# nitishthatte/QuadrotorILQR

Hardware: AMD Instinct MI355X
Metric: iLQR solves/sec (batch, 100-knot SE(3) quadrotor) (higher is better)
Workload: dtype f64

## Files before the change

### profiles/microbench/round_stamps.py

```python
#!/usr/bin/env python3
import ctypes as C, os, sys
import numpy as np
ROOT = os.path.dirname(os.path.dirname(os.path.dirname(os.path.abspath(__file__))))
sys.path.insert(0, ROOT)
from quadrotorilqr_amd import capi, problems as pb
capi.LIB_PATH = os.path.join(ROOT, "quadrotorilqr_amd", "lib", "libquadrotor_ilqr_roundstamps.so")
B = int(sys.argv[1]) if len(sys.argv) > 1 else 1024
cfg = pb.config2(B=B, N=100, seed=2)
s = capi.from_config(cfg)
s.solve_batch(cfg["init"])
lib = capi.load()
zero = np.zeros((max(B, 8) * 8,), dtype=np.uint64)
lib.qilqr_debug_stamps(s._h, zero.ctypes.data_as(C.c_void_p), C.c_int32(B))
out0 = zero.copy()
res = s.solve_batch(cfg["init"])
lib.qilqr_debug_stamps(s._h, zero.ctypes.data_as(C.c_void_p), C.c_int32(B))
d = (zero - out0).reshape(-1, 32)[: (B + 3) // 4, :4].astype(np.float64)
rounds = d[:, 3]
ok = rounds > 0
live_rounds = np.add.reduceat(np.asarray(res["n_fwd"], dtype=np.float64), np.arange(0, B, 4))
print(f"B = {B}: blocks {ok.sum()}, rounds per block (median) {np.median(rounds[ok]):.0f}, in ticks of s_memtime / 100")
for name, k in (("backward pass", 0), ("rollout (until X_0 is through)", 1), ("behind the rollout", 2)):
    per = d[ok, k] / rounds[ok]
    print(f"  {name:32s} median {np.median(per) / 100:7.2f} us per round   (p10 {np.percentile(per, 10) / 100:.2f}, p90 {np.percentile(per, 90) / 100:.2f})")
dense = live_rounds[ok] / rounds[ok]
for lo, hi in ((0.9, 1.5), (1.5, 2.5), (2.5, 4.1)):
    m = (dense >= lo) & (dense < hi)
    if m.sum():
        tot = d[ok][m, :3].sum(axis=1) / rounds[ok][m]
        print(f"  blocks with {lo:.1f}-{hi:.1f} running trajectories per round on average: {m.sum():4d} blocks, {np.median(tot) / 100:7.2f} us per round "
              f"(backward {np.median(d[ok][m, 0] / rounds[ok][m]) / 100:.2f}, rollout {np.median(d[ok][m, 1] / rounds[ok][m]) / 100:.2f}, behind {np.median(d[ok][m, 2] / rounds[ok][m]) / 100:.2f})")
```

### quadrotorilqr_amd/csrc/backward4_body.inc

```
  const int lane = threadIdx.x & 63;
  const int w = __builtin_amdgcn_readfirstlane((int)(threadIdx.x >> 6));
  const int b0 = xcd_local_block(blockIdx.x, gridDim.x) * 4;
#ifndef BW4_LDS_DECLARED
  BW4_DECLARE_LDS
#endif
  if (FREE && threadIdx.x < 24) prog[threadIdx.x] = (threadIdx.x >= 8) ? -1 : 0;
  const RecLayout L = st.layout;

  double mu = 0.0;
  if (w < 4) {
    const int b = b0 + w;
    bool run = false;
    int cur = 0, iters_now = 0, act = 0;
    double cost_now = 0.0;
    if (b < B) {
      int fl = st.flags[b];
      cur = st.cur[b];
      const int it0 = st.iters[b];
      const int trial0 = st.trial[b];
      const double prev_cost0 = st.prev_cost[b], alpha0 = st.alpha[b];
      const double term0 = st.terms[2 * b], term1 = st.terms[2 * b + 1];
      cost_now = st.cost[b];
      const int n_fwd0 = st.n_fwd[b];
      mu = (p.mu_init > 0.0) ? st.mu[b] : 0.0;
      double kc_early[2][2];
#pragma unroll
      for (int h = 0; h < 2; ++h)
#pragma unroll
        for (int k = 0; k < 2; ++k) {
          const int i = 64 * h + lane;
          kc_early[k][h] = (i < n) ? st.knot_cost[k][cost_index(b, i, n)] : 0.0;
        }
      bool restart = false;
      bool settle = false, accept = false, count_active = false, known = true;
      int status = -1;
      double new_cost = 0.0;
      if (!force) {
        if (fl & F_SEARCH) {
          settle = true;
          const double *kc = st.knot_cost[cur ^ 1];
          double *scr = &ring[w][0][0];
          auto add_chunk = [&](double v, int cnt) {
            scr[lane] = v;
            int t = 0;
            for (; t + 8 <= cnt; t += 8) {
              double x[8];
#pragma unroll
              for (int e = 0; e < 8; ++e) x[e] = scr[t + e];
#pragma unroll
              for (int e = 0; e < 8; ++e) new_cost += x[e];
            }
            for (; t < cnt; ++t) new_cost += scr[t];
          };
          add_chunk((cur ^ 1) ? kc_early[1][0] : kc_early[0][0], n < 64 ? n : 64);
          if (n > 64) add_chunk((cur ^ 1) ? kc_early[1][1] : kc_early[0][1], n < 128 ? n - 64 : 64);
          for (int base = 128; base < n; base += 64) {
            const int i = base + lane;
            add_chunk((i < n) ? kc[cost_index(b, i, n)] : 0.0, (n - base < 64) ? n - base : 64);
          }
          if (it0 == 0) {
            accept = true;
          } else {
            const double desired = p.reduction_frac * cost_reduction(term0, term1, alpha0);
            accept = (new_cost - prev_cost0 < desired);
          }
          if (accept) {
            cur ^= 1;
            fl = F_ACTIVE;
            cost_now = new_cost;
            mu = lm_relax(p, mu);
            if (it0 > 0 && is_converged(p, prev_cost0, new_cost)) {
              status = 1;
              fl = 0;
            } else if (!((double)(it0 + 1) < p.max_iters)) {
              status = 2;
              fl = 0;
            }
          } else if (trial0 + 1 >= p.ls_max_iters) {
            if (lm_restart(p, mu)) {
              restart = true;
              fl = F_ACTIVE;
            } else {
              status = 3;
              fl = 0;
            }
          }
          count_active = (fl & F_ACTIVE) != 0;
        } else if (fl == F_ACTIVE) {
          count_active = true;
        } else {
          known = false;
        }
      }
      run = known && (force || !settle || ((accept || restart) && fl != 0));
      iters_now = (settle && accept) ? it0 + 1 : it0;
      if (lane == 0 && known) {
        if (settle) {
          if (p.mu_init > 0.0) st.mu[b] = mu;
          st.n_fwd[b] = n_fwd0 + 1;
          store_settled(st, b, accept, cur, new_cost, it0, trial0, alpha0, p.step_update, status, fl);
        }
        act = count_active ? 1 : 0;
      }
    }
    if (lane == 0) {
      s_act[w] = act;
      s_run[w] = run ? 1 : 0;
      s_cur[w] = cur;
      s_iters[w] = iters_now;
      s_cost[w] = cost_now;
      s_mu[w] = mu;
    }
  }
  __syncthreads();
  const int block_act = s_act[0] + s_act[1] + s_act[2] + s_act[3];
  if ((s_run[0] | s_run[1] | s_run[2] | s_run[3]) == 0) {
    if (threadIdx.x == 0 && block_act) atomicAdd(active_counter(st), block_act);
    BW4_RETURN;
  }

#ifndef BW4_CTAB_FILLED
  bw4_fill_ctab<S>(ring, st.ctab, FUSED ? 320 : 384);
#endif
  if (!FUSED && w == 4) {
    const int g = lane >> 4, j = lane & 15;
    const int bg = (b0 + g < B) ? b0 + g : B - 1;
    const bool grun = s_run[g] != 0;
    double QuTk;
    if constexpr (GFAC) {
      const double cuu_ab = 2.0 * c.R[(j >> 2) * 4 + (j & 3)] + (((j >> 2) == (j & 3)) ? s_mu[g] : 0.0);
      QuTk = bw4f_gradient_wave<S>(ring, kf, kw, L, (S *)st.gains + knot_base<true>(bg, n, 52), (S *)st.dump + 4 * (long)bg, grun, cuu_ab, n, lane);
    } else {
      QuTk = bw4_gradient_wave<S>(ring, kf, L, (S *)st.gains + knot_base<true>(bg, n, 52), (S *)st.dump + 4 * (long)bg, grun, n, lane);
    }
    if (j == 0 && grun) {
      const int b = b0 + g;
      st.terms[2 * b] = QuTk;
      st.terms[2 * b + 1] = -QuTk;
      st.n_bwd[b] += 1;
      if (!force) arm_line_search(p, st, b, s_iters[g], s_cost[g], QuTk, -QuTk);
    }
    if (lane == 0 && block_act) atomicAdd(active_counter(st), block_act);
    BW4_RETURN;
  }

  if (w == (FUSED ? 4 : 5)) {
    const int first = s_run[0] ? 0 : (s_run[1] ? 1 : (s_run[2] ? 2 : 3));
    const S *rec[4];
#pragma unroll
    for (int g = 0; g < 4; ++g) {
      const int gs = s_run[g] ? g : first;
      rec[g] = (const S *)st.lin[s_cur[gs]] + rec_base(L, b0 + gs, n);
    }
    bw4_loader_wave<S, FREE, GFAC>(ring, L, rec[0], rec[1], rec[2], rec[3], n, lane, prog, s_run[0] | (s_run[1] << 1) | (s_run[2] << 2) | (s_run[3] << 3));
    if (FUSED && lane == 0 && block_act) atomicAdd(active_counter(st), block_act);
    if (FREE && lane == 0 && bw4_prog_read(prog, 5) && st.host_error)
      __hip_atomic_store(st.host_error, (2ull << 32) | (unsigned)blockIdx.x, __ATOMIC_RELAXED, __HIP_MEMORY_SCOPE_SYSTEM);
    BW4_RETURN;
  }
  if constexpr (FUSED) {
    const int b = (b0 + w < B) ? b0 + w : B - 1;
    const int j = lane & 15, kk = lane >> 4;
    const bool run = s_run[w] != 0;
    const double cuu = (j >= 12) ? 2.0 * c.R[kk * 4 + (j - 12)] + ((j - 12 == kk) ? mu : 0.0) : 0.0;
    const double QuTk = bw4_fused_wave<S>(ring, L, w, run, (S *)st.gains + knot_base<true>(b, n, 52), (S *)st.dump + 4 * (long)b, cuu, n, lane, prog,
                                          st.stamps ? st.stamps + (long)(b0 + w) * 8 : nullptr);
    if (FREE && lane == 0 && bw4_prog_read(prog, 5) && st.host_error)
      __hip_atomic_store(st.host_error, (2ull << 32) | (unsigned)blockIdx.x, __ATOMIC_RELAXED, __HIP_MEMORY_SCOPE_SYSTEM);
    if (lane == 0 && run) {
      st.terms[2 * b] = QuTk;
      st.terms[2 * b + 1] = -QuTk;
      st.n_bwd[b] += 1;
      if (!force) arm_line_search(p, st, b, s_iters[w], s_cost[w], QuTk, -QuTk);
    }
    BW4_RETURN;
  }
  {
    const int b = (b0 + w < B) ? b0 + w : B - 1;
    const int j = lane & 15, kk = lane >> 4;
    const double cuu = (j >= 12) ? 2.0 * c.R[kk * 4 + (j - 12)] + ((j - 12 == kk) ? mu : 0.0) : 0.0;
#ifndef QILQR_BW4_UNROLL_MANY
#define QILQR_BW4_UNROLL_MANY 1
#endif
    if constexpr (GFAC)
      bw4f_matrix_wave<S, (WAVES >= 6) && QILQR_BW4_UNROLL_MANY>(ring, kf, kw, L, w, s_run[w] != 0, (S *)st.gains + knot_base<true>(b, n, 52),
                                                                (S *)st.dump + 4 * (long)b, cuu, n, lane, st.stamps ? st.stamps + (long)(b0 + w) * 8 : nullptr);
    else
      bw4_matrix_wave<S, (WAVES >= 6) && QILQR_BW4_UNROLL_MANY>(ring, kf, L, w, s_run[w] != 0, (S *)st.gains + knot_base<true>(b, n, 52),
                                                               (S *)st.dump + 4 * (long)b, cuu, n, lane, st.stamps ? st.stamps + (long)(b0 + w) * 8 : nullptr);
  }
```

### quadrotorilqr_amd/csrc/kernels_common.h

```cpp
#pragma once

#include <hip/hip_runtime.h>
#include <stdint.h>

#ifdef QILQR_DIAG
#define QILQR_WITH_SOLVE4 1
#define QILQR_WITH_BACKWARD2 1
#endif

#include <type_traits>

#include "backward_layout.h"
#include "rollout16.h"
#include "se3_math.h"

namespace qilqr {

constexpr int COUNT_BASE = 8, COUNT_STRIPES = 64, COUNT_WORDS = COUNT_BASE + COUNT_STRIPES;
constexpr int F_ACTIVE = 1;
constexpr int F_SEARCH = 2;

struct SolveParams {
  double step_update, reduction_frac, rtol, atol, max_iters;
  int ls_max_iters;
  double mu_init, mu_factor, mu_max;
};

struct BatchState {
  void *traj[2];
  void *lin[2];
  RecLayout layout;
  double *knot_cost[2];
  void *gains;
  const void *desired;
  int desired_tiled;
  int *cur;
  double *cost;
  double *prev_cost;
  double *terms;
  double *alpha;
  double *mu;
  int *trial;
  int *flags;
  int *status, *iters, *n_bwd, *n_fwd;
  int *counters;
  unsigned long long *host_active;
  unsigned long long *host_error;
  double *cost_hist;
  int hist_cap;
  const void *ctab;
  void *dump;
  unsigned long long *stamps;
  int *orig;
  int row0;
  int *plan;
  double *dbg_trajs, *dbg_cost;
  int *dbg_seen;
  int dbg_cap;
  int n_sched;
  const double *q_sched;
};

__device__ __forceinline__ int *active_counter(const BatchState &st) {
  return st.counters + COUNT_BASE + (blockIdx.x & (COUNT_STRIPES - 1));
}

typedef double d4 __attribute__((ext_vector_type(4)));
template <typename S>
struct GA {
  typedef const S __attribute__((address_space(1))) *cptr;
  typedef S v2 __attribute__((ext_vector_type(2)));
  typedef v2 __attribute__((address_space(1))) *ptr2;
  typedef const v2 __attribute__((address_space(1))) *cptr2;
};

#ifdef QILQR_STAMPS
#define QSTAMP(slot)                                                                   \
  do {                                                                                 \
    unsigned long long _t;                                                             \
    __builtin_amdgcn_sched_barrier(0);                                                 \
    asm volatile("s_memtime %0\n\ts_waitcnt lgkmcnt(0)" : "=s"(_t)::"memory");        \
    __builtin_amdgcn_sched_barrier(0);                                                 \
    stamp_sum[slot] += _t - stamp_prev;                                                \
    stamp_prev = _t;                                                                   \
  } while (0)
#define QKEEP(x) asm volatile("" ::"v"(x))
#else
#define QSTAMP(slot) do { } while (0)
#define QKEEP(x) do { } while (0)
#endif

__device__ __forceinline__ int xcd_local_block(unsigned hw_block, unsigned ) { return (int)hw_block; }
__device__ __forceinline__ bool is_converged(const SolveParams &p, double cost, double new_cost) {
  if (fabs(cost - new_cost) / fabs(cost) < p.rtol) return true;
  if (fabs(cost - new_cost) < p.atol) return true;
  return false;
}
__device__ __forceinline__ double cost_reduction(double QuTk, double kTQuuk, double step) {
  return step * QuTk + step * step * kTQuuk / 2.0;
}

__device__ __forceinline__ void store_settled(const BatchState &st, int b, bool accept, int cur, double new_cost, int it0, int trial0,
                                              double alpha0, double step_update, int status, int fl) {
  if (accept) {
    st.cur[b] = cur;
    st.cost[b] = new_cost;
    if (st.cost_hist && it0 < st.hist_cap) st.cost_hist[(long)b * st.hist_cap + it0] = new_cost;
    st.iters[b] = it0 + 1;
  }
  st.trial[b] = accept ? trial0 : trial0 + 1;
  st.alpha[b] = accept ? alpha0 : alpha0 * step_update;
  if (status >= 0) st.status[b] = status;
  st.flags[b] = fl;
}
__device__ __forceinline__ void arm_line_search(const SolveParams &p, const BatchState &st, int b, int iters_now, double cost_now,
                                                double QuTk, double kTQuuk) {
  st.prev_cost[b] = cost_now;
  const bool conv = iters_now > 0 && is_converged(p, cost_now, cost_now + cost_reduction(QuTk, kTQuuk, 1.0));
  const bool none = !conv && iters_now > 0 && p.ls_max_iters <= 0;
  const bool search = !(conv || none);
  st.alpha[b] = 1.0;
  st.trial[b] = 0;
  if (!search) st.status[b] = conv ? 0 : 3;
  st.flags[b] = search ? (F_ACTIVE | F_SEARCH) : 0;
}

}
```

### quadrotorilqr_amd/csrc/rollout16_body.inc

```
  using namespace r16;
  const int lane = threadIdx.x & 63;
  const int role = __builtin_amdgcn_readfirstlane((int)(threadIdx.x >> 6));
  const int row = lane >> 4;
  const int blk = xcd_local_block(blockIdx.x, gridDim.x);
  const int b = blk * 4 + row;
  const int bq = b < B ? b : 0;
  const int fl_own = st.flags[bq], cur_own = st.cur[bq];
  const double alpha_own = st.alpha[bq];
  const bool live = (b < B) && (!need_flag || (fl_own & need_flag));
  const unsigned long long livemask = __ballot(live);
  if (livemask == 0ull) R16_RETURN;
  const int first_live = (__ffsll((long long)livemask) - 1) >> 4;
  const int bs = live ? b : blk * 4 + first_live;
  const int src_lane = (live ? row : first_live) << 4;
  const int cur = __shfl(cur_own, src_lane);
  const double alpha = __shfl(alpha_own, src_lane);
  const S *traj = (const S *)st.traj[cur] + knot_base<true>(bs, n, 18);
  const S *gains = (const S *)st.gains + knot_base<true>(bs, n, 52);
  S *out = (S *)st.traj[cur ^ 1] + knot_base<true>(bs, n, 18);
#ifndef R16_LDS_DECLARED
  __shared__ R16Lds sh;
#endif
  if (threadIdx.x < R16_NFLAGS) sh.flags[threadIdx.x] = 0;
#ifndef R16_LDS_DECLARED
  if (threadIdx.x < 64) r16_exp2_lds[threadIdx.x >> 4][threadIdx.x & 15] = Series<double>::exp2[threadIdx.x >> 4][threadIdx.x & 15];
#endif
  __syncthreads();
#ifdef R16_FOLLOW
  unsigned long long *stamps = (st.stamps && role < 3) ? st.stamps + ((long)blk * 3 + role) * 8 : nullptr;
  if (role == 2) {
    r16_wave_P<S>(sh, traj, gains, out, alpha, live, n, lane, stamps);
  } else if (role < 2) {
    __builtin_amdgcn_s_setprio(3);
    auto ld0 = [&](int e) -> double { return e >= 0 ? (double)traj[knot_elem<true>(0, e, 18)] : 0.0; };
    const double TT = ld0(tt_elem(lane)), QQ = ld0(qq_elem(lane)), VL = ld0(vl_elem(lane)), VW = ld0(vw_elem(lane));
    R16_LOADS_DONE();
    r16_wave_X<S, 2>(sh, c, role, TT, QQ, VL, VW, out, live, n, lane, stamps);
    if (__builtin_expect(r16_flag_read(sh, R16_F_ABORT) != 0, 0) && lane == 0 && st.host_error)
      __hip_atomic_store(st.host_error, (1ull << 32) | (unsigned)blk, __ATOMIC_RELAXED, __HIP_MEMORY_SCOPE_SYSTEM);
    __builtin_amdgcn_s_setprio(0);
#ifdef QILQR_ROUND_STAMPS
    if (role == 0 && lane == 0) {
      unsigned long long t;
      asm volatile("s_memtime %0\n\ts_waitcnt lgkmcnt(0)" : "=s"(t)::"memory");
      *(volatile unsigned long long *)&round_stamp_x0 = t;
    }
#endif
  }
  R16_FOLLOW(b, bs, cur ^ 1, live, __popcll(livemask) == 16);
#else
  if (role >= 3) R16_RETURN;
  unsigned long long *stamps = st.stamps ? st.stamps + ((long)blk * 3 + role) * 8 : nullptr;
  if (role == 2) {
    r16_wave_P<S>(sh, traj, gains, out, alpha, live, n, lane, stamps);
    R16_RETURN;
  }
  __builtin_amdgcn_s_setprio(3);
  auto ld0 = [&](int e) -> double { return e >= 0 ? (double)traj[knot_elem<true>(0, e, 18)] : 0.0; };
  const double TT = ld0(tt_elem(lane)), QQ = ld0(qq_elem(lane)), VL = ld0(vl_elem(lane)), VW = ld0(vw_elem(lane));
  R16_LOADS_DONE();
  r16_wave_X<S, 0>(sh, c, role, TT, QQ, VL, VW, out, live, n, lane, stamps);
  if (__builtin_expect(r16_flag_read(sh, R16_F_ABORT) != 0, 0) && lane == 0 && st.host_error)
    __hip_atomic_store(st.host_error, (1ull << 32) | (unsigned)blk, __ATOMIC_RELAXED, __HIP_MEMORY_SCOPE_SYSTEM);
#endif
```

### quadrotorilqr_amd/csrc/round_body.inc

```
#ifdef QILQR_ROUND_STAMPS
  asm volatile("s_memtime %0\n\ts_waitcnt lgkmcnt(0)" : "=s"(rs_t0)::"memory");
  if (threadIdx.x == 0) *(volatile unsigned long long *)&round_stamp_x0 = 0ull;
#endif
  {
    constexpr int WAVES = SIX ? 6 : 5;
    constexpr bool FUSED = !SIX, FREE = !SIX, GFAC = false;
    (void)GFAC;
    const int force = 0;
    (void)WAVES;
#define BW4_RETURN goto QILQR_CAT(backward_done_, ROUND_ID)
#include "backward4_body.inc"
#undef BW4_RETURN
  }
QILQR_CAT(backward_done_, ROUND_ID):
  __syncthreads();
#ifdef QILQR_ROUND_STAMPS
  asm volatile("s_memtime %0\n\ts_waitcnt lgkmcnt(0)" : "=s"(rs_t1)::"memory");
#endif
  ROUND_BEHIND_BACKWARD
  if (st.dbg_seen && blockIdx.x == 0 && (threadIdx.x >> 6) == 4) debug_capture_wave<S>(st, n, threadIdx.x & 63);
#ifndef QILQR_ROUND_NO_FOLLOW
  {
    const int need_flag = F_SEARCH;
#define R16_RETURN goto QILQR_CAT(rollout_done_, ROUND_ID)
#define R16_FOLLOW(b_, bs_, buf_, live_, single_) round_follow<S, LK>(sh, c, qr_w, st, b_, bs_, buf_, live_, single_, n, lane)
#include "rollout16_body.inc"
#undef R16_FOLLOW
#undef R16_RETURN
  }
QILQR_CAT(rollout_done_, ROUND_ID):
  __syncthreads();
#ifdef QILQR_ROUND_STAMPS
  asm volatile("s_memtime %0\n\ts_waitcnt lgkmcnt(0)" : "=s"(rs_t3)::"memory");
  rs_t2 = *(volatile unsigned long long *)&round_stamp_x0;
  if (threadIdx.x == 0 && st.stamps && rs_t2 != 0ull) {
    unsigned long long *o = st.stamps + (long)blockIdx.x * 32;
    o[0] += rs_t1 - rs_t0; o[1] += rs_t2 - rs_t1; o[2] += rs_t3 - rs_t2; o[3] += 1;
  }
#endif
#else
  {
    const int need_flag = F_SEARCH;
#define R16_RETURN goto QILQR_CAT(rollout_done_, ROUND_ID)
#include "rollout16_body.inc"
#undef R16_RETURN
  }
QILQR_CAT(rollout_done_, ROUND_ID):
  __syncthreads();
  linearize_block<S, LK>(c, qr_w, st, (int)blockIdx.x * 4, B, n, 1, F_SEARCH);
  __syncthreads();
#endif
```

### quadrotorilqr_amd/csrc/round_kernels.h

```cpp
#pragma once

#include "backward4_kernel.h"
#include "rollout16_kernel.h"
#include "linearize_kernels.h"

namespace qilqr {

template <typename S>
__global__ __launch_bounds__(320) void k_backward_rollout(ModelConsts<double> c, SolveParams p, BatchState st, int B, int n) {
  {
    constexpr int WAVES = 5;
    constexpr bool FUSED = true, FREE = true, GFAC = false;
    (void)GFAC;
    const int force = 0;
    (void)WAVES;
#define BW4_RETURN goto backward_done
#include "backward4_body.inc"
#undef BW4_RETURN
  }
backward_done:
  __syncthreads();
  if (threadIdx.x >= 192) return;
  {
    const int need_flag = F_SEARCH;
#define R16_RETURN return
#include "rollout16_body.inc"
#undef R16_RETURN
  }
}

template <typename S, int LK>
__device__ __forceinline__ void linearize_block(const ModelConsts<S> &c, const S *qr, const BatchState &st, int b0, int B, int n, int which,
                                                int need_flag) {
  const int lane = threadIdx.x & 63;
  const int wave = __builtin_amdgcn_readfirstlane((int)(threadIdx.x >> 6)), nwaves = (int)(blockDim.x >> 6);
  int l0 = 0, l1 = 0, l2 = 0, l3 = 0, u0 = 0, u1 = 0, u2 = 0, u3 = 0, nl = 0;
#pragma unroll
  for (int g = 0; g < 4; ++g) {
    const int b = b0 + g;
    if (b >= B) continue;
    const int fl = st.flags[b], buf = st.cur[b] ^ which;
    if (need_flag && !(fl & need_flag)) continue;
    if (nl == 0) { l0 = b; u0 = buf; } else if (nl == 1) { l1 = b; u1 = buf; } else if (nl == 2) { l2 = b; u2 = buf; } else { l3 = b; u3 = buf; }
    ++nl;
  }
  if (nl == 0) return;
  const int per = nl * n, wt = (per + 63) >> 6;
  for (int t = wave; t < 2 * wt; t += nwaves) {
    const bool cost_half = t < wt;
    const int r = (cost_half ? t : t - wt) * 64 + lane;
    if (r >= per) continue;
    const int i = (nl == 1) ? r : (nl == 2) ? (r >> 1) : (nl == 3) ? r / 3 : (r >> 2);
    const int g = r - i * nl;
    const int b = (g == 0) ? l0 : (g == 1) ? l1 : (g == 2) ? l2 : l3;
    const int buf = (g == 0) ? u0 : (g == 1) ? u1 : (g == 2) ? u2 : u3;
    S pt[18];
    load_knot<true>((const S *)st.traj[buf] + knot_base<true>(b, n, 18), i, 18, pt);
    S *rec = (S *)st.lin[buf] + rec_base(st.layout, b, n) + rec_elem(st.layout, i, 0);
    if (!cost_half) {
      const TiledRecWriter<S> wd{rec};
      linearize_dynamics(c, pt, wd);
      wd.flush();
    } else {
      const TiledRecWriter<S> w{rec};
      S pd[18];
      if (st.desired_tiled) load_knot<true>((const S *)st.desired + knot_base<true>(b, n, 18), i, 18, pd);
      else load_knot<false>((const S *)st.desired, i, 18, pd);
      const S cost = linearize_cost<LK>(qr, qr + 144, pt, pd, w);
      w.flush();
      st.knot_cost[buf][cost_index(b, i, n)] = (double)cost;
    }
  }
}
template <typename S, int LK>
__device__ __forceinline__ void round_follow(R16Lds &sh, const ModelConsts<S> &c, const S *qr, const BatchState &st, int b, int bs, int buf, bool live,
                                             bool single, int n, int lane) {
  const int per_task = single ? 64 : R16_CHUNK;
  const int groups = (n + per_task - 1) / per_task, ntasks = 2 * groups;
  for (;;) {
    int t = 0;
    if (lane == 0) t = __hip_atomic_fetch_add(&sh.flags[R16_F_TASK], 1, __ATOMIC_RELAXED, __HIP_MEMORY_SCOPE_WORKGROUP);
    t = __builtin_amdgcn_readfirstlane(t);
    if (t >= ntasks) break;
    const bool cost_half = single ? (t < groups) : ((t & 1) == 0);
    const int k0 = (single ? (cost_half ? t : t - groups) : (t >> 1)) * per_task;
    const int need = single ? n : ((k0 + R16_CHUNK < n) ? k0 + R16_CHUNK : n);
    const int m0 = (need - 1) - ((need - 1) & 1), m1 = (need - 1) - (((need - 1) & 1) ^ 1);
    if (!(r16_flag_wait_relaxed(sh, R16_F_K0, m0 + 1, lane) && (m1 < 0 || r16_flag_wait_relaxed(sh, R16_F_K1, m1 + 1, lane)))) break;
    const int i = k0 + (single ? lane : (lane & 15));
    if (!(single || live) || i >= n) continue;
    const int bb = single ? bs : b;
    S pt[18];
    load_knot<true>((const S *)st.traj[buf] + knot_base<true>(bb, n, 18), i, 18, pt);
    S *rec = (S *)st.lin[buf] + rec_base(st.layout, bb, n) + rec_elem(st.layout, i, 0);
    if (!cost_half) {
      const TiledRecWriter<S> wd{rec};
      linearize_dynamics(c, pt, wd);
      wd.flush();
    } else {
      const TiledRecWriter<S> w{rec};
      S pd[18];
      if (st.desired_tiled) load_knot<true>((const S *)st.desired + knot_base<true>(bb, n, 18), i, 18, pd);
      else load_knot<false>((const S *)st.desired, i, 18, pd);
      const S cost = linearize_cost<LK>(qr, qr + 144, pt, pd, w);
      w.flush();
      st.knot_cost[buf][cost_index(bb, i, n)] = (double)cost;
    }
  }
}
__device__ __forceinline__ void publish_active(int *counters, unsigned long long *host_active, int round, int lane) {
  int act = counters[COUNT_BASE + lane];
  counters[COUNT_BASE + lane] = 0;
#pragma unroll
  for (int off = 32; off > 0; off >>= 1) act += __shfl_xor(act, off);
  if (lane == 0)
    __hip_atomic_store(&host_active[round & 7], ((unsigned long long)(unsigned)(round + 1) << 32) | (unsigned)act, __ATOMIC_RELEASE,
                       __HIP_MEMORY_SCOPE_SYSTEM);
}
__global__ void k_publish_active(int *counters, unsigned long long *host_active, int round) {
  publish_active(counters, host_active, round, threadIdx.x & 63);
}
template <int LK, int ROUNDS, bool SIX = false>
__global__ __launch_bounds__(SIX ? 384 : 320) void k_round(ModelConsts<double> c, const ModelConsts<double> *__restrict__ cp, SolveParams p, BatchState st, int B,
                                                int n, int *prev_counters, int prev_round) {
  typedef double S;
  __shared__ double qr_w[160];
  BW4_DECLARE_LDS
  __shared__ R16Lds sh;
#ifdef QILQR_ROUND_STAMPS
  __shared__ unsigned long long round_stamp_x0;
  unsigned long long rs_t0 = 0, rs_t1 = 0, rs_t2 = 0, rs_t3 = 0;
#endif
#define BW4_LDS_DECLARED
#define R16_LDS_DECLARED
#define BW4_CTAB_FILLED
  for (int k = threadIdx.x; k < 160; k += blockDim.x) qr_w[k] = (k < 144) ? cp->Q[k] : cp->R[k - 144];
  if (threadIdx.x < 64) r16_exp2_lds[threadIdx.x >> 4][threadIdx.x & 15] = Series<double>::exp2[threadIdx.x >> 4][threadIdx.x & 15];
  bw4_fill_ctab<S>(ring, st.ctab, SIX ? 384 : 320);
#define ROUND_BEHIND_BACKWARD \
  if (blockIdx.x == 0 && (threadIdx.x >> 6) == 4 && prev_round >= 0) publish_active(prev_counters, st.host_active, prev_round, threadIdx.x & 63);
#define ROUND_ID 0
#include "round_body.inc"
#undef ROUND_ID
#undef ROUND_BEHIND_BACKWARD
#define ROUND_BEHIND_BACKWARD
  if constexpr (ROUNDS > 1) {
#define ROUND_ID 1
#include "round_body.inc"
#undef ROUND_ID
  }
  if constexpr (ROUNDS > 2) {
#define ROUND_ID 2
#include "round_body.inc"
#undef ROUND_ID
#define ROUND_ID 3
#include "round_body.inc"
#undef ROUND_ID
  }
#undef ROUND_BEHIND_BACKWARD
#undef BW4_LDS_DECLARED
#undef R16_LDS_DECLARED
#undef BW4_CTAB_FILLED
}

}
```

Baseline: 225,100.

## Keep per-trajectory solver state and knot costs in LDS across fused rounds

Inside the multi-round fused kernel, each block now holds its four trajectories' scalar solver state (flags, cur, iters, trial, costs, mu, alpha, terms) in a shared-memory seam struct. Later rounds read that struct instead of reloading from global BatchState. The follow-on linearization also writes knot costs into the ring LDS buffer, so the next round's line-search cost sum reads LDS rather than global memory. This removes global round trips at the start of each round, at the cost of more LDS state, more branches, and reliance on the ring buffer not being overwritten between the rollout and the next backward pass.

```diff
diff --git a/profiles/microbench/round_stamps.py b/profiles/microbench/round_stamps.py
--- a/profiles/microbench/round_stamps.py
+++ b/profiles/microbench/round_stamps.py
@@ -4,7 +4,7 @@
 ROOT = os.path.dirname(os.path.dirname(os.path.dirname(os.path.abspath(__file__))))
 sys.path.insert(0, ROOT)
 from quadrotorilqr_amd import capi, problems as pb
-capi.LIB_PATH = os.path.join(ROOT, "quadrotorilqr_amd", "lib", "libquadrotor_ilqr_roundstamps.so")
+capi.LIB_PATH = os.path.join(ROOT, "quadrotorilqr_amd", "lib", "libquadrotor_ilqr_%s.so" % (sys.argv[2] if len(sys.argv) > 2 else "roundstamps"))
 B = int(sys.argv[1]) if len(sys.argv) > 1 else 1024
 cfg = pb.config2(B=B, N=100, seed=2)
 s = capi.from_config(cfg)
diff --git a/quadrotorilqr_amd/csrc/backward4_body.inc b/quadrotorilqr_amd/csrc/backward4_body.inc
--- a/quadrotorilqr_amd/csrc/backward4_body.inc
+++ b/quadrotorilqr_amd/csrc/backward4_body.inc
@@ -14,6 +14,19 @@
     int cur = 0, iters_now = 0, act = 0;
     double cost_now = 0.0;
     if (b < B) {
+#ifdef BW4_ROUND_STATE
+      const bool kept = BW4_ROUND_KEPT, kc_kept = BW4_ROUND_KC_KEPT && n <= ROUND_KC_MAX;
+      int fl = kept ? rseam.fl[w] : st.flags[b];
+      cur = kept ? rseam.cur[w] : st.cur[b];
+      const int it0 = kept ? rseam.iters[w] : st.iters[b];
+      const int trial0 = kept ? rseam.trial[w] : st.trial[b];
+      const double prev_cost0 = kept ? rseam.prev_cost[w] : st.prev_cost[b], alpha0 = kept ? rseam.alpha[w] : st.alpha[b];
+      const double term0 = kept ? rseam.term0[w] : st.terms[2 * b], term1 = kept ? rseam.term1[w] : st.terms[2 * b + 1];
+      cost_now = kept ? rseam.cost[w] : st.cost[b];
+      const int n_fwd0 = kept ? rseam.n_fwd[w] : st.n_fwd[b];
+      mu = kept ? rseam.mu[w] : ((p.mu_init > 0.0) ? st.mu[b] : 0.0);
+#else
+      constexpr bool kc_kept = false;
       int fl = st.flags[b];
       cur = st.cur[b];
       const int it0 = st.iters[b];
@@ -23,14 +36,17 @@
       cost_now = st.cost[b];
       const int n_fwd0 = st.n_fwd[b];
       mu = (p.mu_init > 0.0) ? st.mu[b] : 0.0;
-      double kc_early[2][2];
-#pragma unroll
-      for (int h = 0; h < 2; ++h)
-#pragma unroll
-        for (int k = 0; k < 2; ++k) {
-          const int i = 64 * h + lane;
-          kc_early[k][h] = (i < n) ? st.knot_cost[k][cost_index(b, i, n)] : 0.0;
-        }
+#endif
+      double kc_early[2][2] = {{0.0, 0.0}, {0.0, 0.0}};
+      if (!kc_kept) {
+#pragma unroll
+        for (int h = 0; h < 2; ++h)
+#pragma unroll
+          for (int k = 0; k < 2; ++k) {
+            const int i = 64 * h + lane;
+            kc_early[k][h] = (i < n) ? st.knot_cost[k][cost_index(b, i, n)] : 0.0;
+          }
+      }
       bool restart = false;
       bool settle = false, accept = false, count_active = false, known = true;
       int status = -1;
@@ -40,24 +56,30 @@
           settle = true;
           const double *kc = st.knot_cost[cur ^ 1];
           double *scr = &ring[w][0][0];
-          auto add_chunk = [&](double v, int cnt) {
-            scr[lane] = v;
+#ifdef BW4_ROUND_STATE
+#define BW4_KC_SRC(base_) (kc_kept ? round_kc(ring, w, base_) : scr)
+#else
+#define BW4_KC_SRC(base_) scr
+#endif
+          auto add_chunk = [&](double v, int cnt, const double *src) {
+            if (!kc_kept) scr[lane] = v;
             int t = 0;
             for (; t + 8 <= cnt; t += 8) {
               double x[8];
 #pragma unroll
-              for (int e = 0; e < 8; ++e) x[e] = scr[t + e];
+              for (int e = 0; e < 8; ++e) x[e] = src[t + e];
 #pragma unroll
               for (int e = 0; e < 8; ++e) new_cost += x[e];
             }
-            for (; t < cnt; ++t) new_cost += scr[t];
+            for (; t < cnt; ++t) new_cost += src[t];
           };
-          add_chunk((cur ^ 1) ? kc_early[1][0] : kc_early[0][0], n < 64 ? n : 64);
-          if (n > 64) add_chunk((cur ^ 1) ? kc_early[1][1] : kc_early[0][1], n < 128 ? n - 64 : 64);
+          add_chunk((cur ^ 1) ? kc_early[1][0] : kc_early[0][0], n < 64 ? n : 64, BW4_KC_SRC(0));
+          if (n > 64) add_chunk((cur ^ 1) ? kc_early[1][1] : kc_early[0][1], n < 128 ? n - 64 : 64, BW4_KC_SRC(64));
           for (int base = 128; base < n; base += 64) {
             const int i = base + lane;
-            add_chunk((i < n) ? kc[cost_index(b, i, n)] : 0.0, (n - base < 64) ? n - base : 64);
-          }
+            add_chunk((!kc_kept && i < n) ? kc[cost_index(b, i, n)] : 0.0, (n - base < 64) ? n - base : 64, BW4_KC_SRC(base));
+          }
+#undef BW4_KC_SRC
           if (it0 == 0) {
             accept = true;
           } else {
@@ -94,15 +116,27 @@
       }
       run = known && (force || !settle || ((accept || restart) && fl != 0));
       iters_now = (settle && accept) ? it0 + 1 : it0;
+#ifdef BW4_ROUND_STATE
+      if (lane == 0) round_keep_state(rseam, w, fl, cur, iters_now, trial0, settle ? n_fwd0 + 1 : n_fwd0, prev_cost0, alpha0, term0, term1, cost_now, mu);
+#endif
       if (lane == 0 && known) {
         if (settle) {
           if (p.mu_init > 0.0) st.mu[b] = mu;
           st.n_fwd[b] = n_fwd0 + 1;
+#ifdef BW4_ROUND_STATE
+          round_store_settled(rseam, w, st, b, accept, cur, new_cost, it0, trial0, alpha0, p.step_update, status, fl);
+#else
           store_settled(st, b, accept, cur, new_cost, it0, trial0, alpha0, p.step_update, status, fl);
+#endif
         }
         act = count_active ? 1 : 0;
       }
     }
+#ifdef BW4_ROUND_STATE
+    else if (lane == 0) {
+      round_keep_state(rseam, w, 0, 0, 0, 0, 0, 0.0, 0.0, 0.0, 0.0, 0.0, 0.0);
+    }
+#endif
     if (lane == 0) {
       s_act[w] = act;
       s_run[w] = run ? 1 : 0;
@@ -138,7 +172,12 @@
       st.terms[2 * b] = QuTk;
       st.terms[2 * b + 1] = -QuTk;
       st.n_bwd[b] += 1;
+#ifdef BW4_ROUND_STATE
+      round_keep_terms(rseam, g, QuTk, -QuTk);
+      if (!force) round_arm_line_search(rseam, g, p, st, b, s_iters[g], s_cost[g], QuTk, -QuTk);
+#else
       if (!force) arm_line_search(p, st, b, s_iters[g], s_cost[g], QuTk, -QuTk);
+#endif
     }
     if (lane == 0 && block_act) atomicAdd(active_counter(st), block_act);
     BW4_RETURN;
@@ -171,7 +210,12 @@
       st.terms[2 * b] = QuTk;
       st.terms[2 * b + 1] = -QuTk;
       st.n_bwd[b] += 1;
+#ifdef BW4_ROUND_STATE
+      round_keep_terms(rseam, w, QuTk, -QuTk);
+      if (!force) round_arm_line_search(rseam, w, p, st, b, s_iters[w], s_cost[w], QuTk, -QuTk);
+#else
       if (!force) arm_line_search(p, st, b, s_iters[w], s_cost[w], QuTk, -QuTk);
+#endif
     }
     BW4_RETURN;
   }
diff --git a/quadrotorilqr_amd/csrc/kernels_common.h b/quadrotorilqr_amd/csrc/kernels_common.h
--- a/quadrotorilqr_amd/csrc/kernels_common.h
+++ b/quadrotorilqr_amd/csrc/kernels_common.h
@@ -113,8 +113,8 @@
   if (status >= 0) st.status[b] = status;
   st.flags[b] = fl;
 }
-__device__ __forceinline__ void arm_line_search(const SolveParams &p, const BatchState &st, int b, int iters_now, double cost_now,
-                                                double QuTk, double kTQuuk) {
+__device__ __forceinline__ int arm_line_search(const SolveParams &p, const BatchState &st, int b, int iters_now, double cost_now,
+                                               double QuTk, double kTQuuk) {
   st.prev_cost[b] = cost_now;
   const bool conv = iters_now > 0 && is_converged(p, cost_now, cost_now + cost_reduction(QuTk, kTQuuk, 1.0));
   const bool none = !conv && iters_now > 0 && p.ls_max_iters <= 0;
@@ -122,7 +122,9 @@
   st.alpha[b] = 1.0;
   st.trial[b] = 0;
   if (!search) st.status[b] = conv ? 0 : 3;
-  st.flags[b] = search ? (F_ACTIVE | F_SEARCH) : 0;
+  const int fl = search ? (F_ACTIVE | F_SEARCH) : 0;
+  st.flags[b] = fl;
+  return fl;
 }
 
 }
diff --git a/quadrotorilqr_amd/csrc/rollout16_body.inc b/quadrotorilqr_amd/csrc/rollout16_body.inc
--- a/quadrotorilqr_amd/csrc/rollout16_body.inc
+++ b/quadrotorilqr_amd/csrc/rollout16_body.inc
@@ -4,9 +4,14 @@
   const int row = lane >> 4;
   const int blk = xcd_local_block(blockIdx.x, gridDim.x);
   const int b = blk * 4 + row;
+#ifdef R16_ROUND_STATE
+  const int fl_own = rseam.fl[row], cur_own = rseam.cur[row];
+  const double alpha_own = rseam.alpha[row];
+#else
   const int bq = b < B ? b : 0;
   const int fl_own = st.flags[bq], cur_own = st.cur[bq];
   const double alpha_own = st.alpha[bq];
+#endif
   const bool live = (b < B) && (!need_flag || (fl_own & need_flag));
   const unsigned long long livemask = __ballot(live);
   if (livemask == 0ull) R16_RETURN;
diff --git a/quadrotorilqr_amd/csrc/round_body.inc b/quadrotorilqr_amd/csrc/round_body.inc
--- a/quadrotorilqr_amd/csrc/round_body.inc
+++ b/quadrotorilqr_amd/csrc/round_body.inc
@@ -8,9 +8,17 @@
     (void)GFAC;
     const int force = 0;
     (void)WAVES;
+#define BW4_ROUND_KEPT (ROUND_ID > 0)
+#ifndef QILQR_ROUND_NO_FOLLOW
+#define BW4_ROUND_KC_KEPT (ROUND_ID > 0)
+#else
+#define BW4_ROUND_KC_KEPT false
+#endif
 #define BW4_RETURN goto QILQR_CAT(backward_done_, ROUND_ID)
 #include "backward4_body.inc"
 #undef BW4_RETURN
+#undef BW4_ROUND_KEPT
+#undef BW4_ROUND_KC_KEPT
   }
 QILQR_CAT(backward_done_, ROUND_ID):
   __syncthreads();
@@ -23,7 +31,7 @@
   {
     const int need_flag = F_SEARCH;
 #define R16_RETURN goto QILQR_CAT(rollout_done_, ROUND_ID)
-#define R16_FOLLOW(b_, bs_, buf_, live_, single_) round_follow<S, LK>(sh, c, qr_w, st, b_, bs_, buf_, live_, single_, n, lane)
+#define R16_FOLLOW(b_, bs_, buf_, live_, single_) round_follow<S, LK>(sh, ring, c, qr_w, st, b_, bs_, buf_, live_, single_, n, lane)
 #include "rollout16_body.inc"
 #undef R16_FOLLOW
 #undef R16_RETURN
diff --git a/quadrotorilqr_amd/csrc/round_kernels.h b/quadrotorilqr_amd/csrc/round_kernels.h
--- a/quadrotorilqr_amd/csrc/round_kernels.h
+++ b/quadrotorilqr_amd/csrc/round_kernels.h
@@ -72,9 +72,48 @@
     }
   }
 }
+constexpr int ROUND_KC_MAX = 512;
+struct RoundSeam {
+  int fl[4], cur[4], iters[4], trial[4], n_fwd[4];
+  double prev_cost[4], alpha[4], term0[4], term1[4], cost[4], mu[4];
+};
+__device__ __forceinline__ double *round_kc(double (&ring)[4][4][BW2_BUF], int r, int i) { return &ring[r][i >> 7][i & 127]; }
+static_assert(ROUND_KC_MAX == 4 * BW2_REC && BW2_REC == 128, "a row's knot costs fill the record words of its four ring slots");
+__device__ __forceinline__ void round_keep_state(RoundSeam &rs, int r, int fl, int cur, int iters, int trial, int n_fwd, double prev_cost, double alpha,
+                                                 double term0, double term1, double cost, double mu) {
+  rs.fl[r] = fl;
+  rs.cur[r] = cur;
+  rs.iters[r] = iters;
+  rs.trial[r] = trial;
+  rs.n_fwd[r] = n_fwd;
+  rs.prev_cost[r] = prev_cost;
+  rs.alpha[r] = alpha;
+  rs.term0[r] = term0;
+  rs.term1[r] = term1;
+  rs.cost[r] = cost;
+  rs.mu[r] = mu;
+}
+__device__ __forceinline__ void round_keep_terms(RoundSeam &rs, int r, double term0, double term1) {
+  rs.term0[r] = term0;
+  rs.term1[r] = term1;
+}
+__device__ __forceinline__ void round_store_settled(RoundSeam &rs, int r, const BatchState &st, int b, bool accept, int cur, double new_cost, int it0,
+                                                    int trial0, double alpha0, double step_update, int status, int fl) {
+  store_settled(st, b, accept, cur, new_cost, it0, trial0, alpha0, step_update, status, fl);
+  rs.trial[r] = accept ? trial0 : trial0 + 1;
+  rs.alpha[r] = accept ? alpha0 : alpha0 * step_update;
+}
+__device__ __forceinline__ void round_arm_line_search(RoundSeam &rs, int r, const SolveParams &p, const BatchState &st, int b, int iters_now,
+                                                      double cost_now, double QuTk, double kTQuuk) {
+  rs.fl[r] = arm_line_search(p, st, b, iters_now, cost_now, QuTk, kTQuuk);
+  rs.prev_cost[r] = cost_now;
+  rs.alpha[r] = 1.0;
+  rs.trial[r] = 0;
+}
+
 template <typename S, int LK>
-__device__ __forceinline__ void round_follow(R16Lds &sh, const ModelConsts<S> &c, const S *qr, const BatchState &st, int b, int bs, int buf, bool live,
-                                             bool single, int n, int lane) {
+__device__ __forceinline__ void round_follow(R16Lds &sh, double (&ring)[4][4][BW2_BUF], const ModelConsts<S> &c, const S *qr, const BatchState &st, int b, int bs, int buf,
+                                             bool live, bool single, int n, int lane) {
   const int per_task = single ? 64 : R16_CHUNK;
   const int groups = (n + per_task - 1) / per_task, ntasks = 2 * groups;
   for (;;) {
@@ -105,6 +144,7 @@
       const S cost = linearize_cost<LK>(qr, qr + 144, pt, pd, w);
       w.flush();
       st.knot_cost[buf][cost_index(bb, i, n)] = (double)cost;
+      if (n <= ROUND_KC_MAX) *round_kc(ring, bb & 3, i) = (double)cost;
     }
   }
 }
@@ -127,6 +167,7 @@
   __shared__ double qr_w[160];
   BW4_DECLARE_LDS
   __shared__ R16Lds sh;
+  __shared__ RoundSeam rseam;
 #ifdef QILQR_ROUND_STAMPS
   __shared__ unsigned long long round_stamp_x0;
   unsigned long long rs_t0 = 0, rs_t1 = 0, rs_t2 = 0, rs_t3 = 0;
@@ -134,6 +175,8 @@
 #define BW4_LDS_DECLARED
 #define R16_LDS_DECLARED
 #define BW4_CTAB_FILLED
+#define BW4_ROUND_STATE
+#define R16_ROUND_STATE
   for (int k = threadIdx.x; k < 160; k += blockDim.x) qr_w[k] = (k < 144) ? cp->Q[k] : cp->R[k - 144];
   if (threadIdx.x < 64) r16_exp2_lds[threadIdx.x >> 4][threadIdx.x & 15] = Series<double>::exp2[threadIdx.x >> 4][threadIdx.x & 15];
   bw4_fill_ctab<S>(ring, st.ctab, SIX ? 384 : 320);
@@ -161,6 +204,8 @@
 #undef BW4_LDS_DECLARED
 #undef R16_LDS_DECLARED
 #undef BW4_CTAB_FILLED
-}
-
-}
+#undef BW4_ROUND_STATE
+#undef R16_ROUND_STATE
+}
+
+}
```

After: 226,000 (median of 6 runs). No clear change (+0.4%).
